# nicklashansen/tdmpc2

Hardware: AMD Instinct MI355X
Metric: plan() calls/sec (H=3, 512 samples, 6 iters) (higher is better)
Workload: dtype f32 (f16x2-split products: 22-bit operands, fp32 accumulate)

## Files before the change

tdmpc2_amd/csrc/common.cuh:

```cuda
#pragma once
#include <hip/hip_runtime.h>

#include <cmath>
#include <cstdint>
#include <cstdio>
#include <cstdlib>
#include <cstring>

#include "../../include/tdmpc2_plan.h"
#include "layer_route.h"
#include "plan_layout.h"
#include "fused_route.h"

typedef float f32x16 __attribute__((ext_vector_type(16)));
typedef float f32x4 __attribute__((ext_vector_type(4)));
typedef _Float16 f16x8 __attribute__((ext_vector_type(8)));
typedef _Float16 f16x4 __attribute__((ext_vector_type(4)));

namespace tdk {

constexpr int NTHREADS = 512;
constexpr float LN_EPS = 1e-5f;

constexpr int GBN = 128;
// ... 40 lines not shown
__device__ __forceinline__ void raise_fault(unsigned int *err, unsigned int code) {
    __hip_atomic_store(err, code, __ATOMIC_RELAXED, __HIP_MEMORY_SCOPE_SYSTEM);
    __hip_atomic_store(err + 8, 1u, __ATOMIC_RELAXED, __HIP_MEMORY_SCOPE_SYSTEM);
}

struct RefitParams {
    int E, N, H, A, K, iter, last, eval_mode;
    int Nvalid;
    int stage;
    float temperature, min_std, max_std;
    float *value;
    const float *actions;
    const float *act_mask;
    float *mean, *std;
    float *score;
    int *elite_idx;
    const float *gumbel_exp;
    const float *final_eps;
    unsigned long long seed;
    unsigned int call;
    float *prev_mean;
    float *action;
    const unsigned int *err;
    const unsigned int *err2;
    int regen, P, Apad;
    const float *sample_eps;
    long sample_eps_estride;
    float *dbg_value; long dbg_value_es;
    int *dbg_idx; long dbg_idx_es;
    float *dbg_score; long dbg_score_es;
    float *dbg_mean; long dbg_mean_es;
    float *dbg_std; long dbg_std_es;
};

struct RolloutParams {
    int E, N, H, A, Apad, P, stride, tiles, nq, num_bins, multitask, given_actions, iter, iters_total;
    int tile_off;
    int nnets;
    float log_std_min, log_std_dif;
    NetS dyn, rew, pi, term;
    NetS q[MAXQ];
    const float *bins;
    const float *z0;
    const float *beff;
    const float *cvec;
    const float *act_mask;
    const float *disc_pow;
    const float *mean;
    const float *std;
    const float *sample_eps;
    long sample_eps_estride;
    const float *pi_eps;
    long pi_eps_estride;
    const int *qidx;
    long qidx_estride;
    unsigned long long seed;
    unsigned int call;
    float *actions;
    float *value;
    float *zscratch;
    float *trace_tiles;
    float *trace_scalars;
    unsigned long long *timing;
    int fold_refit;
    unsigned int *ticket;
    RefitParams rf;
// ... 447 lines not shown
```

tdmpc2_amd/csrc/fused_kernels.cuh:

```cuda
#pragma once

#include "kloop_schedule.h"

#ifdef SPLIT_TIMING
#define TIMER_FIELDS mutable unsigned long long t_acc[14] = {0, 0, 0, 0, 0, 0, 0, 0, 0, 0, 0, 0, 0, 0}; mutable unsigned long long t_last = 0, t_begin = 0;
#define TIMER_START(c) { (c).t_last = (c).t_begin = __builtin_amdgcn_s_memtime(); }
#define TIMER_MARK(c, cls) { __builtin_amdgcn_sched_barrier(0); const unsigned long long t_now = __builtin_amdgcn_s_memtime(); __builtin_amdgcn_sched_barrier(0); (c).t_acc[cls] += t_now - (c).t_last; (c).t_last = t_now; }
#ifndef SPLIT_TIMING_WAVE
#define SPLIT_TIMING_WAVE 4
#endif
#define TIMER_FLUSH(c, ptr) if ((ptr) && threadIdx.x == 64 * SPLIT_TIMING_WAVE) { for (int i_ = 0; i_ < 14; ++i_) atomicAdd((ptr) + i_, (c).t_acc[i_]); atomicAdd((ptr) + 14, (c).t_last - (c).t_begin); atomicAdd((ptr) + 15, 1ull); }
#else
#define TIMER_FIELDS
#define TIMER_START(c)
#define TIMER_MARK(c, cls)
#define TIMER_FLUSH(c, ptr)
#endif
enum { T_KLOOP = 0, T_EPI = 1, T_HEAD = 2, T_ACT = 3, T_PARK = 4, T_TILE = 5, T_EPI_PRE = 6, T_EPI_SYNC = 7, T_EPI_BIAS = 8,
       T_EPI_COMB = 9, T_EPI_MATH = 10, T_CL_WAIT = 11, T_HEAD_K = 12, T_HEAD_ST = 13 };



#ifdef KS_NO_BIAS_LDS
constexpr bool KS_BIAS_LDS = false;
#else
constexpr bool KS_BIAS_LDS = true;
#endif
#ifdef KS_NO_ZH_REGS
constexpr bool KS_ZH_REGS = false;
#else
constexpr bool KS_ZH_REGS = true;
#endif
template <int APAD, int ST = 2, int NW = 8, int AR = 0>
struct CtxT {
    static constexpr bool BIAS_LDS = false;
    static constexpr int NST = ST;
    static constexpr int NWAVES = NW;
    static constexpr int ARITH = AR;
    static constexpr int FT = 16 / NW;
    static constexpr int NTHR = 64 * NW;
    static constexpr int TROWS = 32 * ST;
    static constexpr int SH = WIDTH + APAD;
    static constexpr int RSH = 2 * SH + 8;
    static constexpr int RSF_ = AR == 0 ? RSH / 2 : WIDTH + APAD + 4;
    static constexpr int KBLK = AR == 0 ? 16 : 8;
    static constexpr int ZKB = WIDTH / KBLK;
    _Float16 *act;
    float *stats;
    float *gb;
    int tid, wave, lane;
    mutable float pg[(WIDTH + NTHR - 1) / NTHR], pb[(WIDTH + NTHR - 1) / NTHR];
    TIMER_FIELDS
    __device__ __forceinline__ float *f32() const { return reinterpret_cast<float *>(act); }
    static constexpr __device__ __forceinline__ int RSF() { return RSF_; }
};
template <int APAD, int ST, int NW, int AR>
struct CtxPhT : CtxT<APAD, ST, NW, AR> {
    static constexpr bool BIAS_LDS = KS_BIAS_LDS;
    mutable float pbias = 0.f;
};

__device__ __forceinline__ float mish_fast(float x) {
    const float e = __expf(fminf(x, 20.f));
    const float n = e * (e + 2.f);
    return x * (n * __builtin_amdgcn_rcpf(n + 2.f));
}

template <class CT>
__device__ __forceinline__ float exp_a(float x) {
    if constexpr (CT::ARITH == 1) return expf(x);
    else return __expf(x);
}
template <class CT>
__device__ __forceinline__ float mish_a(float x) {
    if constexpr (CT::ARITH == 1) {
        const float e = expf(fminf(x, 20.f));
        const float n = e * (e + 2.f);
        return x * (n / (n + 2.f));
    } else {
        return mish_fast(x);
    }
}

__device__ __forceinline__ void split4(const f32x4 y, f16x4 &hi, f16x4 &lo, const float scale = ACT_SCALE) {
#pragma unroll
    for (int e = 0; e < 4; ++e) {
        const float ys = y[e] * scale;
        const _Float16 h = (_Float16)ys;
        hi[e] = h;
        lo[e] = (_Float16)(ys - (float)h);
    }
}


constexpr int PF = 2;
template <int FT>
struct BFragT {
    f16x8 h[FT], l[FT];
};
__device__ __forceinline__ f16x8 ldw(const char *ubase, unsigned voff, int imm) {
    return *reinterpret_cast<const f16x8 *>(ubase + voff + imm);
}
#define SPLIT_MFMA(a, b, c) __builtin_amdgcn_mfma_f32_32x32x16_f16(a, b, c, 0, 0, 0)
template <int FT>
__device__ __forceinline__ void load_b(BFragT<FT> &b, const char *u0, size_t ct_stride, unsigned voff) {
#pragma unroll
    for (int cc = 0; cc < FT; ++cc) {
        b.h[cc] = ldw(u0 + cc * ct_stride, voff, 0);
        b.l[cc] = ldw(u0 + cc * ct_stride, voff, 1024);
    }
}
template <int ST, int FT>
__device__ __forceinline__ void zero_acc(f32x16 (&a)[ST][FT]) {
#pragma unroll
    for (int r = 0; r < ST; ++r)
#pragma unroll
        for (int cc = 0; cc < FT; ++cc)
#pragma unroll
            for (int e = 0; e < 16; ++e) a[r][cc][e] = 0.f;
}
template <int ST>
struct AFragT {
    f16x8 h[ST], l[ST];
};
template <class CT>
__device__ __forceinline__ void load_a(AFragT<CT::NST> &a, const _Float16 *a0p, int kk) {
#pragma unroll
    for (int st = 0; st < CT::NST; ++st) {
        a.h[st] = *reinterpret_cast<const f16x8 *>(a0p + st * 32 * CT::RSH + kk * 16);
        a.l[st] = *reinterpret_cast<const f16x8 *>(a0p + st * 32 * CT::RSH + CT::SH + kk * 16);
    }
}
// ... 62 lines not shown
    a_dsrd<0>(a.h[0], la0);
    a_dsrd<2 * CT::SH>(a.l[0], la0);
    if constexpr (CT::NST == 2) {
        a_dsrd<0>(a.h[1], la1);
        a_dsrd<2 * CT::SH>(a.l[1], la1);
    }
}
__device__ __forceinline__ void a_load_w(BFragT<2> &b, unsigned voff, const char *s0, const char *s1) {
    asm volatile("s_nop 4\n\t"
                 "global_load_dwordx4 %0, %4, %5\n\t"
                 "global_load_dwordx4 %1, %4, %5 offset:1024\n\t"
                 "global_load_dwordx4 %2, %4, %6\n\t"
                 "global_load_dwordx4 %3, %4, %6 offset:1024"
                 : "=&v"(b.h[0]), "=&v"(b.l[0]), "=&v"(b.h[1]), "=&v"(b.l[1])
                 : "v"(voff), "s"(s0), "s"(s1));
}
template <class CT>
__device__ __forceinline__ void a_mfma12(f32x16 (&acc)[CT::NST][2], const BFragT<2> &w, const AFragT<CT::NST> &a) {
#pragma unroll
    for (int cc = 0; cc < 2; ++cc)
#pragma unroll
        for (int st = 0; st < CT::NST; ++st) A_MFMA(acc[st][cc], w.h[cc], a.h[st]);
#pragma unroll
    for (int cc = 0; cc < 2; ++cc)
#pragma unroll
        for (int st = 0; st < CT::NST; ++st) A_MFMA(acc[st][cc], w.l[cc], a.h[st]);
#pragma unroll
    for (int cc = 0; cc < 2; ++cc)
#pragma unroll
        for (int st = 0; st < CT::NST; ++st) A_MFMA(acc[st][cc], w.h[cc], a.l[st]);
}

template <class CT>
__device__ __forceinline__ void kloop_asm(const CT &c, const LayerS &ly, int kb0, int kb1, f32x16 (&acc)[CT::NST][2]) {
    static_assert(CT::FT == 2 && CT::ARITH == 0, "hand-ordered loop: 8-wave split-arithmetic geometry");
    const int i = c.lane & 31, hh = c.lane >> 5;
    unsigned la0 = lds_addr_of(c.act) + (unsigned)((i * CT::RSH + 8 * hh + kb0 * 16) * 2);
    unsigned la1 = la0 + 32 * CT::RSH * 2;
    const char *u0 = reinterpret_cast<const char *>(ly.wp) + ((size_t)(2 * c.wave) * ly.KB + kb0) * 2048;
    const size_t cts = (size_t)ly.KB * 2048;
    const unsigned voff = (unsigned)c.lane * 16u;
    const int nk = kb1 - kb0;
    constexpr int RD = KL_RD;
    BFragT<2> ring[RD];
    AFragT<CT::NST> a2[2];
#pragma unroll
    for (int d = 0; d < RD; ++d)
        if (d < nk) a_load_w(ring[d], voff, u0 + d * 2048, u0 + cts + d * 2048);
    a_load_act<CT>(a2[0], la0, la1);
    int k = 0;
    const char *pn = u0 + RD * 2048;
#pragma unroll 1
    for (; kl_steady_trip(k, nk, RD); k += RD) {
#pragma unroll
        for (int d = 0; d < RD; ++d) {
            asm volatile("s_waitcnt lgkmcnt(0)" ::: "memory");
            la0 += 32;
            la1 += 32;
            a_load_act<CT>(a2[(d & 1) ^ 1], la0, la1);
            asm volatile("s_waitcnt vmcnt(4)" ::: "memory");
            a_mfma12<CT>(acc, ring[d], a2[d & 1]);
            a_load_w(ring[d], voff, pn, pn + cts);
            pn += 2048;
        }
    }
#pragma unroll 1
    for (; k < nk; k += RD) {
#pragma unroll
        for (int d = 0; d < RD; ++d) {
            const int kk = k + d;
            if (kk < nk) {
                asm volatile("s_waitcnt lgkmcnt(0)" ::: "memory");
                if (kl_next_act(kk, nk)) {
                    la0 += 32;
                    la1 += 32;
                    a_load_act<CT>(a2[(d & 1) ^ 1], la0, la1);
                }
                const int behind = kl_behind(kk, nk, RD);
                if (behind >= 5) asm volatile("s_waitcnt vmcnt(20)" ::: "memory");
                else if (behind == 4) asm volatile("s_waitcnt vmcnt(16)" ::: "memory");
                else if (behind == 3) asm volatile("s_waitcnt vmcnt(12)" ::: "memory");
                else if (behind == 2) asm volatile("s_waitcnt vmcnt(8)" ::: "memory");
                else if (behind == 1) asm volatile("s_waitcnt vmcnt(4)" ::: "memory");
                else asm volatile("s_waitcnt vmcnt(0)" ::: "memory");
                a_mfma12<CT>(acc, ring[d], a2[d & 1]);
                if (kl_issue(kk, nk, RD)) {
                    a_load_w(ring[d], voff, pn, pn + cts);
                    pn += 2048;
                }
            }
        }
    }
    asm volatile("s_nop 7\n\ts_nop 7" ::: "memory");
}

template <class CT>
__device__ __forceinline__ void kloop_s(const CT &c, const LayerS &ly, int kb0, int kb1, f32x16 (&acc)[CT::NST][CT::FT]) {
    if constexpr (CT::ARITH == 1) {
        kloop_f32(c, ly, kb0, kb1, acc);
        return;
    }
    if constexpr (CT::ARITH == 0 && CT::FT == 2) {
        kloop_asm(c, ly, kb0, kb1, acc);
        return;
    }
    constexpr int FT = CT::FT;
    constexpr int PFD = FT == 2 ? PF : (PF > 1 ? PF / 2 : 1);
    const int i = c.lane & 31, hh = c.lane >> 5;
    const _Float16 *a0p = c.act + i * c.RSH + 8 * hh + kb0 * 16;
    const char *u0 = reinterpret_cast<const char *>(ly.wp) + ((size_t)(FT * c.wave) * ly.KB + kb0) * 2048;
    const size_t cts = (size_t)ly.KB * 2048;
    unsigned voff = (unsigned)c.lane * 16u;
    asm volatile("" : "+v"(voff));
    const int nk = kb1 - kb0;
    BFragT<FT> ring[PFD];
#pragma unroll
    for (int d = 0; d < PFD; ++d) {
        const int kd = d < nk ? d : nk - 1;
        load_b(ring[d], u0 + (size_t)kd * 2048, cts, voff);
    }
    AFragT<CT::NST> an;
    load_a<CT>(an, a0p, 0);
    __builtin_amdgcn_sched_barrier(0);
#pragma unroll 1
    for (int k = 0; k < nk; k += PFD) {
#pragma unroll
        for (int d = 0; d < PFD; ++d) {
            const int kk = k + d;
            if (kk < nk) {
                const AFragT<CT::NST> a = an;
                load_a<CT>(an, a0p, kk + 1 < nk ? kk + 1 : kk);
#pragma unroll
                for (int cc = 0; cc < FT; ++cc)
#pragma unroll
                    for (int st = 0; st < CT::NST; ++st) acc[st][cc] = SPLIT_MFMA(ring[d].h[cc], a.h[st], acc[st][cc]);
#pragma unroll
// ... 163 lines not shown
        _Float16 *hp = c.act + (32 * st + j) * c.RSH + 32 * CT::FT * c.wave + 4 * hh;
#pragma unroll
        for (int ft = 0; ft < CT::FT; ++ft)
#pragma unroll
            for (int m = 0; m < 4; ++m) {
                f32x4 v;
#pragma unroll
                for (int r = 0; r < 4; ++r) v[r] = y[st][ft][4 * m + r];
                f16x4 hi, lo;
                split4(v, hi, lo, scale);
                *reinterpret_cast<f16x4 *>(hp + 32 * ft + 8 * m) = hi;
                *reinterpret_cast<f16x4 *>(hp + c.SH + 32 * ft + 8 * m) = lo;
            }
    }
}

struct GB {
    const float *g = nullptr, *b = nullptr, *bias = nullptr;
};
__device__ __forceinline__ GB gb_of(const LayerS &ly) { return GB{ly.g, ly.b, ly.bias}; }
__device__ __forceinline__ GB gb_of(const LayerS &ly, const float *bias) { return GB{ly.g, ly.b, bias}; }

template <class CT>
__device__ __forceinline__ void gb_prefetch(const CT &c, const float *g, const float *b) {
#pragma unroll
    for (int u = 0; u < (WIDTH + CT::NTHR - 1) / CT::NTHR; ++u) {
        const int f = c.tid + u * CT::NTHR;
        c.pg[u] = f < WIDTH ? g[f] : 0.f;
        c.pb[u] = f < WIDTH ? b[f] : 0.f;
    }
}
template <class CT>
__device__ __forceinline__ void gb_prefetch(const CT &c, const GB next) {
    gb_prefetch(c, next.g, next.b);
    if constexpr (CT::BIAS_LDS) {
        static_assert(CT::FT == 2 && CT::NTHR == WIDTH, "thread tid fetches feature tid of its own wave's 64");
        c.pbias = next.bias[c.tid];
    }
}
template <class CT>
__device__ __forceinline__ void gb_commit(const CT &c) {
    if constexpr (CT::BIAS_LDS) c.stats[c.wave * (CT::TROWS * 2) + c.lane] = c.pbias;
#pragma unroll
    for (int u = 0; u < (WIDTH + CT::NTHR - 1) / CT::NTHR; ++u) {
        const int f = c.tid + u * CT::NTHR;
        if (f < WIDTH) {
            c.gb[f] = c.pg[u];
            c.gb[WIDTH + f] = c.pb[u];
        }
    }
}
template <class CT>
__device__ __forceinline__ void epi_barrier(const CT &c) {
    __syncthreads();
    gb_commit(c);
}

enum { EPI_PRE = 1, EPI_MATH = 2, EPI_STORE = 4, EPI_ALL = 7 };
template <int ACT, class CT, bool HASBIAS = true, int PIECES = EPI_ALL>
__device__ __forceinline__ void epi_t(const CT &c, f32x16 (&acc)[CT::NST][CT::FT], float osc, float asc, const float *bias,
                                      GB next, float *zcopy) {
    constexpr int FT = CT::FT, NW = CT::NWAVES;
    constexpr float CNT = 32.f * FT;
    const int j = c.lane & 31, hh = c.lane >> 5;
    const int poff = 32 * FT * c.wave + 4 * hh;
    if constexpr (PIECES & EPI_PRE) {
// ... 161 lines not shown

template <class CT>
__device__ __forceinline__ float twohot_rows_s(const CT &c, const float *bins, int num_bins) {
    const int part = c.tid & 7;
    const bool live = (c.tid >> 3) < CT::TROWS;
    const int row = live ? c.tid >> 3 : 0;
    const float *rp = c.f32() + row * c.RSF();
    if (num_bins <= 1) {
        const float x1 = rp[0];
        return num_bins == 0 ? x1 : symexp_f(x1);
    }
    float v[16];
    float m = -INFINITY;
#pragma unroll
    for (int q = 0; q < 16; ++q) {
        const int jj = part + 8 * q;
        v[q] = (jj < num_bins) ? rp[jj] : -INFINITY;
        m = fmaxf(m, v[q]);
    }
    m = group_max<8>(m);
    float es = 0.f, x = 0.f;
#pragma unroll
    for (int q = 0; q < 16; ++q) {
        const int jj = part + 8 * q;
        const float ev = (jj < num_bins) ? expf(v[q] - m) : 0.f;
        es += ev;
        x = fmaf(ev, (jj < num_bins) ? bins[jj] : 0.f, x);
    }
    es = group_sum<8>(es);
    x = group_sum<8>(x);
    return symexp_f(x / es);
}

template <int ACT, class CT>
__device__ __forceinline__ void layer_full_s(const CT &c, const LayerS &ly, const float *bias, int kb0, int kb1,
                                             GB next, float *zcopy = nullptr) {
    f32x16 acc[CT::NST][CT::FT];
    zero_acc(acc);
    if (next.g) gb_prefetch(c, next);
    kloop_s(c, ly, kb0, kb1, acc);
    TIMER_MARK(c, T_KLOOP)
    epi_t<ACT>(c, acc, *ly.oscale, *ly.ascale, bias, next, zcopy);
    epi_barrier(c);
    TIMER_MARK(c, T_EPI)
}
template <int ACT, class CT>
__device__ __forceinline__ void layer_held_s(const CT &c, const LayerS &ly, const float *bias, int kb0, int kb1, GB next,
                                             f32x16 (&acc)[CT::NST][CT::FT]) {
    zero_acc(acc);
    if (next.g) gb_prefetch(c, next);
    kloop_s(c, ly, kb0, kb1, acc);
    TIMER_MARK(c, T_KLOOP)
    epi_t<ACT>(c, acc, *ly.oscale, *ly.ascale, bias, next, nullptr);
    epi_barrier(c);
    TIMER_MARK(c, T_EPI)
}

template <class CT>
__device__ __forceinline__ void head_logits_s(const CT &c, const LayerS &ly) {
    f32x16 acc[CT::NST];
    const float osc = *ly.oscale;
    const int ct = c.wave;
    if (ct < ly.CT) kloop_tile_s(c, ly, ct, 0, CT::ZKB, acc);
    __syncthreads();
    TIMER_MARK(c, T_HEAD_K)
    if (ct < ly.CT) {
#pragma unroll
        for (int rt = 0; rt < CT::NST; ++rt) store_tile_s(c, acc[rt], osc, ly.bias, ct, rt);
    }
    __syncthreads();
    TIMER_MARK(c, T_HEAD_ST)
}

template <class CT>
__device__ __forceinline__ float head_twohot_s(const CT &c, const LayerS &ly, const float *bins, int num_bins) {
    head_logits_s(c, ly);
    const float r = twohot_rows_s(c, bins, num_bins);
    __syncthreads();
    return r;
}

template <class CT>
__device__ __forceinline__ void put_action(const CT &c, int row, int a, float v) {
    if constexpr (CT::ARITH == 1) {
        c.f32()[row * CT::RSF() + WIDTH + a] = v;
        return;
    }
    const float vs = v * ACT_SCALE;
    const _Float16 h = (_Float16)vs;
    _Float16 *rp = c.act + row * c.RSH + WIDTH + a;
    rp[0] = h;
    rp[c.SH] = (_Float16)(vs - (float)h);
}

template <class CT, typename EpsFn>
__device__ __forceinline__ void head_pi_rows_s(const CT &c, int A, int Apad, float lsmin, float lsdif, const float *mask_wg, EpsFn eps,
                                               float *gdst, int nvalid, float *tsc, const float *mask_tab = nullptr,
                                               const int *row_task = nullptr, int put_rows = CT::TROWS, bool agent_store = false);

template <class CT, typename EpsFn>
__device__ __forceinline__ void head_pi_s(const CT &c, const LayerS &ly, int A, int Apad, float lsmin, float lsdif,
                                          const float *mask_wg, EpsFn eps, float *gdst, int nvalid, float *tsc,
                                          const float *mask_tab = nullptr, const int *row_task = nullptr) {
    head_logits_s(c, ly);
    head_pi_rows_s(c, A, Apad, lsmin, lsdif, mask_wg, eps, gdst, nvalid, tsc, mask_tab, row_task, CT::TROWS, false);
}

template <class CT, typename EpsFn>
__device__ __forceinline__ void head_pi_rows_s(const CT &c, int A, int Apad, float lsmin, float lsdif, const float *mask_wg, EpsFn eps,
                                               float *gdst, int nvalid, float *tsc, const float *mask_tab, const int *row_task,
// ... 234 lines not shown
#pragma unroll
        for (int u = 0; u < 2; ++u) {
            const int a = a0 + u;
            if (a < p.A) {
                if (!sampled) {
                    v[u] = ag[(size_t)n * p.A + a];
                } else {
                    float r = z[u];
                    if (p.sample_eps)
                        r = p.sample_eps[(size_t)e * p.sample_eps_estride +
                                         (unsigned)(((size_t)t * (p.N - p.P) + (n - p.P)) * p.A + a)];
                    v[u] = sample_action(sm_mean[t * p.A + a], sm_std[t * p.A + a], r);
                }
                if (mask && !p.given_actions) v[u] *= mask[a];
                if (!p.given_actions) ag[(size_t)n * p.A + a] = v[u];
            }
            put_action(c, row, a, v[u]);
        }
    }
}

#define DUMP_TILE(...) do { if constexpr (TRACE) dump_tile_s(__VA_ARGS__); } while (0)
template <int APAD, int ST, int NW, int AR, int EP, int TR = 0>
__global__ __launch_bounds__(64 * NW, 2) void ks_rollout(RolloutParams p) {
    constexpr bool TRACE = TR || EP;
    extern __shared__ __attribute__((aligned(16))) float smem[];
    __shared__ int s_is_last;
    const int e = blockIdx.x / p.tiles, tile = p.tile_off + blockIdx.x % p.tiles;
    const int tid = threadIdx.x;
    typedef CtxPhT<APAD, ST, NW, AR> CT;
    constexpr int TROWS = CT::TROWS, NTHR = CT::NTHR, FT = CT::FT;
    constexpr int ZKB16 = CT::ZKB;
    constexpr bool ZH_REGS = !EP && KS_ZH_REGS;
    CT c{{reinterpret_cast<_Float16 *>(smem), smem + TROWS * CT::RSF(), smem + TROWS * CT::RSF() + 1024, tid,
          __builtin_amdgcn_readfirstlane(tid >> 6), tid & 63}};
    float *sm_mean = smem + TROWS * CT::RSF() + 2048;
    float *sm_std = sm_mean + p.H * p.A;
    const int row0 = tile * TROWS;
    const float *mask = p.act_mask ? p.act_mask + (size_t)e * p.A : nullptr;
    const float *disc = p.disc_pow + (size_t)e * (p.H + 1);
    const int KBA = ZKB16 + p.Apad / CT::KBLK;
    float *zs = p.zscratch + (size_t)blockIdx.x * TROWS * WIDTH;
    const int NSLOT = 5 * p.H + 7;
    const bool live = (tid >> 3) < TROWS;
    float *tsc = nullptr;
    if constexpr (TRACE) tsc = p.trace_scalars && live ? p.trace_scalars + ((size_t)e * p.N + row0 + (tid >> 3)) * (p.H + 2 + p.A) : nullptr;

    for (int idx = tid; idx < p.H * p.A; idx += NTHR) {
        sm_mean[idx] = p.mean[(size_t)e * p.H * p.A + idx];
        sm_std[idx] = p.std[(size_t)e * p.H * p.A + idx];
    }
    int q0, q1;
    if (p.qidx) {
        q0 = p.qidx[(size_t)e * p.qidx_estride + 0];
        q1 = p.qidx[(size_t)e * p.qidx_estride + 1];
    } else {
        const uint4 r = rng_raw(p.seed, p.call, SITE_QIDX, p.iter, e, 0);
        q0 = (int)(r.x % (unsigned)p.nq);
        q1 = (int)(r.y % (unsigned)(p.nq - 1));
        if (q1 >= q0) ++q1;
    }
    const float *b_rew = p.multitask ? p.beff + ((size_t)e * p.nnets + BE_REW) * WIDTH : p.rew.l[0].bias;
    const float *b_dyn = p.multitask ? p.beff + ((size_t)e * p.nnets + BE_DYN) * WIDTH : p.dyn.l[0].bias;
    const float *b_pi = p.multitask ? p.beff + ((size_t)e * p.nnets + BE_PI) * WIDTH : p.pi.l[0].bias;
    const float *b_q0 = p.multitask ? p.beff + ((size_t)e * p.nnets + BE_Q0 + q0) * WIDTH : p.q[q0].l[0].bias;
    const float *b_q1 = p.multitask ? p.beff + ((size_t)e * p.nnets + BE_Q0 + q1) * WIDTH : p.q[q1].l[0].bias;
    const float *c_rew = p.cvec + ((size_t)e * 2 + 0) * WIDTH, *c_dyn = p.cvec + ((size_t)e * 2 + 1) * WIDTH;
    gb_prefetch(c, gb_of(p.rew.l[0], c_rew));
    epi_barrier(c);

    float G = 0.f;
    float termv = 0.f;
    TIMER_START(c)
    for (int t = 0; t < p.H; ++t) {
        sample_actions(c, p, e, row0, mask, sm_mean, sm_std, t);
        __syncthreads();
        TIMER_MARK(c, T_ACT)
        const bool term_step = EP && t > 0;
        f32x16 accd[ST][FT];
        {
            f32x16 acc[ST][FT];
            gb_prefetch(c, gb_of(p.rew.l[1]));
            first_layers_s(c, p.dyn.l[0], p.rew.l[0], t == 0 ? ZKB16 : 0, KBA, accd, acc);
            TIMER_MARK(c, T_KLOOP)
            if constexpr (EP) {
                if (term_step) {
                    park(c, accd, zs);
                    zero_acc(accd);
                    kloop_s(c, p.term.l[0], 0, ZKB16, accd);
                }
            }
            epi_t<0>(c, acc, *p.rew.l[0].oscale, *p.rew.l[0].ascale, t == 0 ? c_rew : b_rew, gb_of(p.rew.l[1]), nullptr);
        }
        epi_barrier(c);
        TIMER_MARK(c, T_EPI)
        DUMP_TILE(c, p.trace_tiles, NSLOT, 5 * t + 0, p.rew.l[0].ascale);
        layer_full_s<0>(c, p.rew.l[1], p.rew.l[1].bias, 0, ZKB16,
                        term_step ? gb_of(p.term.l[0]) : gb_of(p.dyn.l[0], t == 0 ? c_dyn : b_dyn));
        DUMP_TILE(c, p.trace_tiles, NSLOT, 5 * t + 1, p.rew.l[1].ascale);
        if (term_step) gb_prefetch(c, gb_of(p.term.l[1]));
        else gb_prefetch(c, gb_of(p.dyn.l[1]));
        const float r = head_twohot_s(c, p.rew.l[2], p.bins, p.num_bins);
        TIMER_MARK(c, T_HEAD)
        if (tsc && (tid & 7) == 0) tsc[t] = r;
        if constexpr (EP) {
            if (term_step) {
                epi_t<0>(c, accd, *p.term.l[0].oscale, *p.term.l[0].ascale, p.term.l[0].bias, gb_of(p.term.l[1]), nullptr);
                epi_barrier(c);
                layer_full_s<0>(c, p.term.l[1], p.term.l[1].bias, 0, ZKB16, gb_of(p.dyn.l[0], b_dyn));
                gb_prefetch(c, gb_of(p.dyn.l[1]));
                termv = fminf(termv + head_term_s(c, p.term.l[2]), 1.f);
                unpark(c, accd, zs);
            }
        }
        G += disc[t] * (1.f - termv) * r;
        epi_t<0>(c, accd, *p.dyn.l[0].oscale, *p.dyn.l[0].ascale, t == 0 ? c_dyn : b_dyn, gb_of(p.dyn.l[1]), nullptr);
        epi_barrier(c);
        TIMER_MARK(c, T_EPI)
        DUMP_TILE(c, p.trace_tiles, NSLOT, 5 * t + 2, p.dyn.l[0].ascale);
        layer_full_s<0>(c, p.dyn.l[1], p.dyn.l[1].bias, 0, ZKB16, gb_of(p.dyn.l[2]));
        DUMP_TILE(c, p.trace_tiles, NSLOT, 5 * t + 3, p.dyn.l[1].ascale);
        if constexpr (ZH_REGS) {
            if (t == p.H - 1) break;
            layer_full_s<1>(c, p.dyn.l[2], p.dyn.l[2].bias, 0, ZKB16, gb_of(p.rew.l[0], b_rew), nullptr);
        } else {
            layer_full_s<1>(c, p.dyn.l[2], p.dyn.l[2].bias, 0, ZKB16,
                            t == p.H - 1 ? gb_of(p.pi.l[0], b_pi) : gb_of(p.rew.l[0], b_rew), t == p.H - 1 ? zs : nullptr);
        }
        DUMP_TILE(c, p.trace_tiles, NSLOT, 5 * t + 4);
    }
    f32x16 acch[ST][FT];
    if constexpr (ZH_REGS) {
        layer_held_s<1>(c, p.dyn.l[2], p.dyn.l[2].bias, 0, ZKB16, gb_of(p.pi.l[0], b_pi), acch);
        DUMP_TILE(c, p.trace_tiles, NSLOT, 5 * (p.H - 1) + 4);
    }
    if constexpr (EP) {
        zero_acc(acch);
        kloop_s(c, p.term.l[0], 0, ZKB16, acch);
    }
    layer_full_s<0>(c, p.pi.l[0], b_pi, 0, ZKB16, gb_of(p.pi.l[1]));
    DUMP_TILE(c, p.trace_tiles, NSLOT, 5 * p.H + 0, p.pi.l[0].ascale);
    layer_full_s<0>(c, p.pi.l[1], p.pi.l[1].bias, 0, ZKB16, EP ? gb_of(p.term.l[0]) : gb_of(p.q[q0].l[0], b_q0));
    DUMP_TILE(c, p.trace_tiles, NSLOT, 5 * p.H + 1, p.pi.l[1].ascale);
    if constexpr (EP) gb_prefetch(c, gb_of(p.term.l[1]));
    {
        auto eps = [&](int row, int a) -> float {
            const unsigned ridx = (unsigned)((size_t)(row0 + row) * p.A + a);
            if (p.pi_eps) return p.pi_eps[(size_t)e * p.pi_eps_estride + ridx];
            return rng_normal(p.seed, p.call, SITE_PI, p.iter, e, ridx);
        };
        head_pi_s(c, p.pi.l[2], p.A, p.Apad, p.log_std_min, p.log_std_dif, mask, eps, nullptr, 0,
                  tsc ? tsc + p.H + 2 : nullptr);
    }
    TIMER_MARK(c, T_HEAD)
    if constexpr (EP) {
        epi_t<0>(c, acch, *p.term.l[0].oscale, *p.term.l[0].ascale, p.term.l[0].bias, gb_of(p.term.l[1]), nullptr);
        epi_barrier(c);
        layer_full_s<0>(c, p.term.l[1], p.term.l[1].bias, 0, ZKB16, gb_of(p.q[q0].l[0], b_q0));
        termv = fminf(termv + head_term_s(c, p.term.l[2]), 1.f);
    }
    if constexpr (ZH_REGS) regs_to_tile(c, acch);
    else tile_from_global_s(c, zs);
    __syncthreads();
    TIMER_MARK(c, T_TILE)
    DUMP_TILE(c, p.trace_tiles, NSLOT, 5 * p.H + 2);
    {
        f32x16 acc[ST][FT];
        gb_prefetch(c, gb_of(p.q[q0].l[1]));
        first_layers_s(c, p.q[q1].l[0], p.q[q0].l[0], 0, KBA, acch, acc);
        TIMER_MARK(c, T_KLOOP)
        epi_t<0>(c, acc, *p.q[q0].l[0].oscale, *p.q[q0].l[0].ascale, b_q0, gb_of(p.q[q0].l[1]), nullptr);
    }
    epi_barrier(c);
    TIMER_MARK(c, T_EPI)
    DUMP_TILE(c, p.trace_tiles, NSLOT, 5 * p.H + 3, p.q[q0].l[0].ascale);
    layer_full_s<0>(c, p.q[q0].l[1], p.q[q0].l[1].bias, 0, ZKB16, gb_of(p.q[q1].l[0], b_q1));
    DUMP_TILE(c, p.trace_tiles, NSLOT, 5 * p.H + 4, p.q[q0].l[1].ascale);
    gb_prefetch(c, gb_of(p.q[q1].l[1]));
    const float qa = head_twohot_s(c, p.q[q0].l[2], p.bins, p.num_bins);
    TIMER_MARK(c, T_HEAD)
    epi_t<0>(c, acch, *p.q[q1].l[0].oscale, *p.q[q1].l[0].ascale, b_q1, gb_of(p.q[q1].l[1]), nullptr);
    epi_barrier(c);
    TIMER_MARK(c, T_EPI)
    DUMP_TILE(c, p.trace_tiles, NSLOT, 5 * p.H + 5, p.q[q1].l[0].ascale);
    layer_full_s<0>(c, p.q[q1].l[1], p.q[q1].l[1].bias, 0, ZKB16, GB{});
    DUMP_TILE(c, p.trace_tiles, NSLOT, 5 * p.H + 6, p.q[q1].l[1].ascale);
    const float qb = head_twohot_s(c, p.q[q1].l[2], p.bins, p.num_bins);
    TIMER_MARK(c, T_HEAD)
    TIMER_FLUSH(c, p.timing)
    if (tsc && (tid & 7) == 0) {
        tsc[p.H] = qa;
        tsc[p.H + 1] = qb;
    }
    const float val = G + disc[p.H] * (1.f - termv) * ((qa + qb) / 2.f);
    if (!p.fold_refit) {
        if ((tid & 7) == 0 && live) p.value[(size_t)e * p.N + row0 + (tid >> 3)] = val;
        return;
    }
    if ((tid & 7) == 0 && live)
        __hip_atomic_store(p.value + (size_t)e * p.N + row0 + (tid >> 3), val, __ATOMIC_RELAXED, __HIP_MEMORY_SCOPE_AGENT);
    asm volatile("s_waitcnt vmcnt(0)" ::: "memory");
    __builtin_amdgcn_fence(__ATOMIC_RELEASE, "workgroup");
    __syncthreads();
    if (tid == 0) {
        const unsigned old = __hip_atomic_fetch_add(p.ticket + e, 1u, __ATOMIC_RELAXED, __HIP_MEMORY_SCOPE_AGENT);
        const int last = old == (unsigned)(p.tiles - 1);
        if (last) __hip_atomic_store(p.ticket + e, 0u, __ATOMIC_RELAXED, __HIP_MEMORY_SCOPE_AGENT);
        s_is_last = last;
    }
    __syncthreads();
    if (!s_is_last) return;
    refit_plan(p.rf, e, smem, tid, NTHR);
}

template <int APAD, int AR>
__global__ __launch_bounds__(NTHREADS, 2) void ks_value(ValueParams p) {
    extern __shared__ __attribute__((aligned(16))) float smem[];
    const int tid = threadIdx.x;
// ... 73 lines not shown
```

tdmpc2_amd/csrc/kloop_schedule.h:

```cpp
#pragma once

#ifndef __HIPCC__
#ifndef __host__
#define __host__
#endif
#ifndef __device__
#define __device__
#endif
#endif

constexpr int KL_RD = 2;
constexpr int KL_W_LOADS = 4;

__host__ __device__ inline bool kl_steady_trip(int k, int nk, int rd) { return k + 2 * rd - 1 < nk; }
__host__ __device__ inline int kl_steady_vmcnt(int rd) { return KL_W_LOADS * (rd - 1); }
__host__ __device__ inline int kl_behind(int kk, int nk, int rd) { return nk - 1 - kk < rd - 1 ? nk - 1 - kk : rd - 1; }
__host__ __device__ inline bool kl_next_act(int kk, int nk) { return kk + 1 < nk; }
__host__ __device__ inline bool kl_issue(int kk, int nk, int rd) { return kk + rd < nk; }
```

tdmpc2_amd/csrc/tdmpc2_plan.hip:

```cpp
#include <cstdarg>
#include <cstring>
#include <new>

#include "handle.h"
#include "launch.h"

namespace {

__global__ void k_refit(RefitParams p) {
    extern __shared__ __attribute__((aligned(16))) float smem[];
    refit_plan(p, blockIdx.x, smem, threadIdx.x, blockDim.x);
}

}
int tdk::launch_refit(const RefitParams &fp, int E, int N, size_t lds, hipStream_t st) {
    hipLaunchKernelGGL(k_refit, dim3(E), dim3(refit_threads(N)), lds, st, fp);
    LAUNCH_CHECK();
    return 0;
}
namespace {

__global__ void ks_task_bias(TaskBiasParams p) {
    const int task = blockIdx.x, f = threadIdx.x;
    const float *emb = p.task_emb + (size_t)task * p.T;
// ... 651 lines not shown
        L.side = sr.stream; L.ev_fork = sr.ev[0]; L.ev_side = sr.ev[1]; L.ev_xread = sr.ev[2];
    }
    if (lo.err_line && (rc = err_line_create(h))) return rc;
    if (hipEventCreateWithFlags(&h->turn_ev, hipEventDisableTiming) != hipSuccess) {
        h->turn_ev = nullptr;
        return fail(TDMPC2_ERR_HIP, "hipEventCreate failed");
    }
    if (pl_set_lds()) return TDMPC2_ERR_HIP;
    if (!L.on) {
        const int ar = h->split ? 0 : 1;
        rc = fused_ops(h->Apad).set_lds(ar, c.episodic, h->lds_bytes);
        if (!rc) rc = model_ops(h->Apad).set_lds(ar, h->lds_bytes);
        if (!rc) rc = policy_loss_ops(h->Apad).set_lds(ar, h->lds_bytes);
        if (!rc && h->cl_max_clusters) rc = cluster_ops(h->Apad).set_lds(c.episodic, h->cl_lds);
        if (rc) return TDMPC2_ERR_HIP;
    }
    if (L.on && h->split) {
        L.fuse_ln = env.fuse_ln;
        L.ksplit = env.ksplit;
        L.mid = env.fewrow;
        if ((rc = ksws_ensure(h, L.ksplit))) return rc;
        if (env.gw_timing) {
            if ((rc = dev_alloc(h, (void **)&L.gw_timing, 32 * 8))) return rc;
            if (hipMemset(L.gw_timing, 0, 32 * 8) != hipSuccess) return fail(TDMPC2_ERR_HIP, "hipMemset failed");
        }
    }
    h->cluster_mode = env.cluster;
    h->user_cluster_mode = h->cluster_mode;
    h->user_fuse_ln = L.fuse_ln;
#ifdef TDMPC2_TEST_HOOKS
    if (const char *cf = getenv("TDMPC2_CLUSTER_FAULT")) h->cl_fault = atoi(cf);
#endif
    if (h->cl_fault) L.mid = false;
    if (env.timing && dev_alloc(h, (void **)&h->timing, 16 * 8) == 0) (void)hipMemset(h->timing, 0, 16 * 8);
    undo.h = nullptr;
    *out = h;
    return TDMPC2_OK;
}

void tdmpc2_plan_destroy(tdmpc2_plan_t *h) {
    if (!h) return;
    DevGuard dev_(h->cfg.device);
    if (h->timing) {
        unsigned long long t[16];
        if (hipMemcpy(t, h->timing, sizeof t, hipMemcpyDeviceToHost) == hipSuccess && t[15] > 0) {
            static const char *names[16] = {"kloop", "epi_post", "head", "actions", "park/unpark", "tile_from_global", "epi_stats", "epi_sync",
                                            "epi_bias", "epi_combine", "epi_math_store", "cluster_wait", "head_kloop", "head_stage", "total", "workgroups"};
            fprintf(stderr, "[tdmpc2_plan timing max_envs=%d] mean cycles per workgroup (one wave, SPLIT_TIMING_WAVE):", h->cfg.max_envs);
            for (int i = 0; i < 15; ++i)
                if (names[i][0]) fprintf(stderr, " %s=%.0f", names[i], (double)t[i] / (double)t[15]);
            fprintf(stderr, "\n");
        }
    }
    if (h->lay.gw_timing) {
        unsigned long long t[32];
        if (hipDeviceSynchronize() == hipSuccess && hipMemcpy(t, h->lay.gw_timing, sizeof t, hipMemcpyDeviceToHost) == hipSuccess) {
            static const char *cls[4] = {"mish K<1024", "mish K>=1024", "simnorm K<1024", "simnorm K>=1024"};
            for (int c = 0; c < 4; ++c) {
                const unsigned long long *q = t + 8 * c;
                if (!q[6]) continue;
                const double n = (double)q[6];
                fprintf(stderr, "[g_gemm_w timing max_envs=%d, %s] workgroups=%llu mean cycles of wave 0: loop_end=%.0f stats_stored=%.0f "
                        "peers_arrived=%.0f row_stats=%.0f end=%.0f\n", h->cfg.max_envs, cls[c], q[6], q[1] / n, q[2] / n, q[3] / n, q[4] / n, q[5] / n);
            }
        }
    }
    if (h->lay.side) {
        SideRes sr;
        sr.stream = h->lay.side; sr.ev[0] = h->lay.ev_fork; sr.ev[1] = h->lay.ev_side; sr.ev[2] = h->lay.ev_xread;
        side_release(h->cfg.device, sr);
    }
    for (void *p : h->allocs) (void)hipFree(p);
    if (h->cl_err_host) (void)hipHostFree(h->cl_err_host);
    for (hipEvent_t e : h->ev) (void)hipEventDestroy(e);
    if (h->turn_ev) (void)hipEventDestroy(h->turn_ev);
    delete h;
}

uint64_t tdmpc2_plan_device_bytes(const tdmpc2_plan_t *h) { return h ? h->bytes : 0; }
int tdmpc2_plan_path(const tdmpc2_plan_t *h) { return h ? h->cfg.path : -1; }
int tdmpc2_plan_precision(const tdmpc2_plan_t *h) { return h ? h->cfg.precision : -1; }

namespace {
// ... 1504 lines not shown
```

Before: 10350.

## Prefetch next layer's weight ring during epilogue across layer seams

Moves the initial weight-block ring loads of the hand-ordered k-loop into a per-context ring that is issued during the previous layer's epilogue, before the barrier, so global weight loads for the next layer overlap epilogue math and the sync. It also loads gamma/beta/bias prefetch with a single per-thread address (SEAM_ADDR) instead of the generic path. It extends split timing with new counter classes. The ring now lives across function boundaries, which raises register pressure and risks spills or lower occupancy.

```diff
diff --git a/tdmpc2_amd/csrc/common.cuh b/tdmpc2_amd/csrc/common.cuh
--- a/tdmpc2_amd/csrc/common.cuh
+++ b/tdmpc2_amd/csrc/common.cuh
@@ -96,6 +96,8 @@
     float *dbg_mean; long dbg_mean_es;
     float *dbg_std; long dbg_std_es;
 };
+
+constexpr int T_NCLS = 17;
 
 struct RolloutParams {
     int E, N, H, A, Apad, P, stride, tiles, nq, num_bins, multitask, given_actions, iter, iters_total;
diff --git a/tdmpc2_amd/csrc/fused_kernels.cuh b/tdmpc2_amd/csrc/fused_kernels.cuh
--- a/tdmpc2_amd/csrc/fused_kernels.cuh
+++ b/tdmpc2_amd/csrc/fused_kernels.cuh
@@ -3,13 +3,13 @@
 #include "kloop_schedule.h"
 
 #ifdef SPLIT_TIMING
-#define TIMER_FIELDS mutable unsigned long long t_acc[14] = {0, 0, 0, 0, 0, 0, 0, 0, 0, 0, 0, 0, 0, 0}; mutable unsigned long long t_last = 0, t_begin = 0;
+#define TIMER_FIELDS mutable unsigned long long t_acc[T_NCLS] = {}; mutable unsigned long long t_last = 0, t_begin = 0;
 #define TIMER_START(c) { (c).t_last = (c).t_begin = __builtin_amdgcn_s_memtime(); }
 #define TIMER_MARK(c, cls) { __builtin_amdgcn_sched_barrier(0); const unsigned long long t_now = __builtin_amdgcn_s_memtime(); __builtin_amdgcn_sched_barrier(0); (c).t_acc[cls] += t_now - (c).t_last; (c).t_last = t_now; }
 #ifndef SPLIT_TIMING_WAVE
 #define SPLIT_TIMING_WAVE 4
 #endif
-#define TIMER_FLUSH(c, ptr) if ((ptr) && threadIdx.x == 64 * SPLIT_TIMING_WAVE) { for (int i_ = 0; i_ < 14; ++i_) atomicAdd((ptr) + i_, (c).t_acc[i_]); atomicAdd((ptr) + 14, (c).t_last - (c).t_begin); atomicAdd((ptr) + 15, 1ull); }
+#define TIMER_FLUSH(c, ptr) if ((ptr) && threadIdx.x == 64 * SPLIT_TIMING_WAVE) { for (int i_ = 0; i_ < T_NCLS; ++i_) atomicAdd((ptr) + i_, (c).t_acc[i_]); atomicAdd((ptr) + T_NCLS, (c).t_last - (c).t_begin); atomicAdd((ptr) + T_NCLS + 1, 1ull); }
 #else
 #define TIMER_FIELDS
 #define TIMER_START(c)
@@ -17,7 +17,9 @@
 #define TIMER_FLUSH(c, ptr)
 #endif
 enum { T_KLOOP = 0, T_EPI = 1, T_HEAD = 2, T_ACT = 3, T_PARK = 4, T_TILE = 5, T_EPI_PRE = 6, T_EPI_SYNC = 7, T_EPI_BIAS = 8,
-       T_EPI_COMB = 9, T_EPI_MATH = 10, T_CL_WAIT = 11, T_HEAD_K = 12, T_HEAD_ST = 13 };
+       T_EPI_COMB = 9, T_EPI_MATH = 10, T_CL_WAIT = 11, T_HEAD_K = 12, T_HEAD_ST = 13,
+       T_KLOOP_HEAD = 14, T_EPI_OSC = 15, T_TWOHOT = 16 };
+static_assert(T_TWOHOT + 1 == T_NCLS, "common.cuh: T_NCLS counters + total + workgroups");
 
 
 
@@ -31,9 +33,24 @@
 #else
 constexpr bool KS_ZH_REGS = true;
 #endif
+#ifdef KS_NO_SEAM_WARM
+constexpr bool KS_SEAM_RING = false;
+#else
+constexpr bool KS_SEAM_RING = true;
+#endif
+#ifdef KS_NO_SEAM_ADDR
+constexpr bool KS_SEAM_ADDR = false;
+#else
+constexpr bool KS_SEAM_ADDR = true;
+#endif
+template <int FT>
+struct BFragT {
+    f16x8 h[FT], l[FT];
+};
 template <int APAD, int ST = 2, int NW = 8, int AR = 0>
 struct CtxT {
     static constexpr bool BIAS_LDS = false;
+    static constexpr bool SEAM_RING = false, SEAM_ADDR = false;
     static constexpr int NST = ST;
     static constexpr int NWAVES = NW;
     static constexpr int ARITH = AR;
@@ -57,7 +74,10 @@
 template <int APAD, int ST, int NW, int AR>
 struct CtxPhT : CtxT<APAD, ST, NW, AR> {
     static constexpr bool BIAS_LDS = KS_BIAS_LDS;
+    static constexpr bool SEAM_RING = KS_SEAM_RING && AR == 0 && NW == 8;
+    static constexpr bool SEAM_ADDR = KS_SEAM_ADDR;
     mutable float pbias = 0.f;
+    mutable BFragT<2> ring[KL_RD];
 };
 
 __device__ __forceinline__ float mish_fast(float x) {
@@ -94,10 +114,6 @@
 
 
 constexpr int PF = 2;
-template <int FT>
-struct BFragT {
-    f16x8 h[FT], l[FT];
-};
 __device__ __forceinline__ f16x8 ldw(const char *ubase, unsigned voff, int imm) {
     return *reinterpret_cast<const f16x8 *>(ubase + voff + imm);
 }
@@ -226,8 +242,26 @@
 }
 
 template <class CT>
+__device__ __forceinline__ void ring_issue(const CT &c, const LayerS &ly, int kb0, int kb1) {
+    static_assert(CT::SEAM_RING && CT::FT == 2 && CT::ARITH == 0, "the hand-ordered loop's ring");
+    const char *wp = reinterpret_cast<const char *>(ly.wp);
+    const unsigned voff = (unsigned)c.lane * 16u;
+    const int nk = kb1 - kb0;
+#pragma unroll
+    for (int d = 0; d < KL_RD; ++d)
+        if (kl_ring_fill(d, nk, KL_RD))
+            a_load_w(c.ring[d], voff, wp + kl_block_offset(2 * c.wave, ly.KB, kb0 + d), wp + kl_block_offset(2 * c.wave + 1, ly.KB, kb0 + d));
+}
+template <bool PRE, class CT>
+__device__ __forceinline__ auto &ring_of(const CT &c, BFragT<2> (&local)[KL_RD]) {
+    if constexpr (PRE) return c.ring;
+    else return local;
+}
+
+template <class CT, bool PRE = false>
 __device__ __forceinline__ void kloop_asm(const CT &c, const LayerS &ly, int kb0, int kb1, f32x16 (&acc)[CT::NST][2]) {
     static_assert(CT::FT == 2 && CT::ARITH == 0, "hand-ordered loop: 8-wave split-arithmetic geometry");
+    TIMER_MARK(c, T_KLOOP)
     const int i = c.lane & 31, hh = c.lane >> 5;
     unsigned la0 = lds_addr_of(c.act) + (unsigned)((i * CT::RSH + 8 * hh + kb0 * 16) * 2);
     unsigned la1 = la0 + 32 * CT::RSH * 2;
@@ -236,12 +270,20 @@
     const unsigned voff = (unsigned)c.lane * 16u;
     const int nk = kb1 - kb0;
     constexpr int RD = KL_RD;
-    BFragT<2> ring[RD];
+    BFragT<2> lring[RD];
+    BFragT<2> (&ring)[RD] = ring_of<PRE>(c, lring);
     AFragT<CT::NST> a2[2];
-#pragma unroll
-    for (int d = 0; d < RD; ++d)
-        if (d < nk) a_load_w(ring[d], voff, u0 + d * 2048, u0 + cts + d * 2048);
+    if constexpr (!PRE) {
+#pragma unroll
+        for (int d = 0; d < RD; ++d)
+            if (kl_ring_fill(d, nk, RD)) a_load_w(ring[d], voff, u0 + d * 2048, u0 + cts + d * 2048);
+    }
     a_load_act<CT>(a2[0], la0, la1);
+#ifdef SPLIT_TIMING
+    if (nk > 1) asm volatile("s_waitcnt lgkmcnt(0)\n\ts_waitcnt vmcnt(4)" ::: "memory");
+    else asm volatile("s_waitcnt lgkmcnt(0)\n\ts_waitcnt vmcnt(0)" ::: "memory");
+    TIMER_MARK(c, T_KLOOP_HEAD)
+#endif
     int k = 0;
     const char *pn = u0 + RD * 2048;
 #pragma unroll 1
@@ -288,14 +330,15 @@
     asm volatile("s_nop 7\n\ts_nop 7" ::: "memory");
 }
 
-template <class CT>
+template <class CT, bool PRE = false>
 __device__ __forceinline__ void kloop_s(const CT &c, const LayerS &ly, int kb0, int kb1, f32x16 (&acc)[CT::NST][CT::FT]) {
+    static_assert(!PRE || (CT::ARITH == 0 && CT::FT == 2), "only the hand-ordered loop takes a ring requested ahead");
     if constexpr (CT::ARITH == 1) {
         kloop_f32(c, ly, kb0, kb1, acc);
         return;
     }
     if constexpr (CT::ARITH == 0 && CT::FT == 2) {
-        kloop_asm(c, ly, kb0, kb1, acc);
+        kloop_asm<CT, PRE>(c, ly, kb0, kb1, acc);
         return;
     }
     constexpr int FT = CT::FT;
@@ -525,6 +568,15 @@
 }
 template <class CT>
 __device__ __forceinline__ void gb_prefetch(const CT &c, const GB next) {
+    if constexpr (CT::BIAS_LDS && CT::SEAM_ADDR) {
+        static_assert(CT::FT == 2 && CT::NTHR == WIDTH, "thread tid fetches feature tid of its own wave's 64");
+        unsigned f = (unsigned)c.tid;
+        asm volatile("" : "+v"(f));
+        c.pg[0] = next.g[f];
+        c.pb[0] = next.b[f];
+        c.pbias = next.bias[f];
+        return;
+    }
     gb_prefetch(c, next.g, next.b);
     if constexpr (CT::BIAS_LDS) {
         static_assert(CT::FT == 2 && CT::NTHR == WIDTH, "thread tid fetches feature tid of its own wave's 64");
@@ -752,26 +804,38 @@
     return symexp_f(x / es);
 }
 
-template <int ACT, class CT>
+#ifdef SPLIT_TIMING
+#define TIMER_MARK_SCALARS(c) { asm volatile("s_waitcnt lgkmcnt(0)" ::: "memory"); TIMER_MARK(c, T_EPI_OSC) }
+#else
+#define TIMER_MARK_SCALARS(c)
+#endif
+
+template <int ACT, class CT, bool PRE = false, bool NK = false>
 __device__ __forceinline__ void layer_full_s(const CT &c, const LayerS &ly, const float *bias, int kb0, int kb1,
-                                             GB next, float *zcopy = nullptr) {
+                                             GB next, float *zcopy = nullptr, const LayerS *nxk = nullptr) {
     f32x16 acc[CT::NST][CT::FT];
     zero_acc(acc);
     if (next.g) gb_prefetch(c, next);
-    kloop_s(c, ly, kb0, kb1, acc);
+    kloop_s<CT, PRE>(c, ly, kb0, kb1, acc);
     TIMER_MARK(c, T_KLOOP)
-    epi_t<ACT>(c, acc, *ly.oscale, *ly.ascale, bias, next, zcopy);
+    const float osc = *ly.oscale, asc = *ly.ascale;
+    TIMER_MARK_SCALARS(c)
+    epi_t<ACT>(c, acc, osc, asc, bias, next, zcopy);
+    if constexpr (NK) ring_issue(c, *nxk, 0, CT::ZKB);
     epi_barrier(c);
     TIMER_MARK(c, T_EPI)
 }
-template <int ACT, class CT>
+template <int ACT, class CT, bool PRE = false, bool NK = false>
 __device__ __forceinline__ void layer_held_s(const CT &c, const LayerS &ly, const float *bias, int kb0, int kb1, GB next,
-                                             f32x16 (&acc)[CT::NST][CT::FT]) {
+                                             f32x16 (&acc)[CT::NST][CT::FT], const LayerS *nxk = nullptr) {
     zero_acc(acc);
     if (next.g) gb_prefetch(c, next);
-    kloop_s(c, ly, kb0, kb1, acc);
+    kloop_s<CT, PRE>(c, ly, kb0, kb1, acc);
     TIMER_MARK(c, T_KLOOP)
-    epi_t<ACT>(c, acc, *ly.oscale, *ly.ascale, bias, next, nullptr);
+    const float osc = *ly.oscale, asc = *ly.ascale;
+    TIMER_MARK_SCALARS(c)
+    epi_t<ACT>(c, acc, osc, asc, bias, next, nullptr);
+    if constexpr (NK) ring_issue(c, *nxk, 0, CT::ZKB);
     epi_barrier(c);
     TIMER_MARK(c, T_EPI)
 }
@@ -796,6 +860,7 @@
 __device__ __forceinline__ float head_twohot_s(const CT &c, const LayerS &ly, const float *bins, int num_bins) {
     head_logits_s(c, ly);
     const float r = twohot_rows_s(c, bins, num_bins);
+    TIMER_MARK(c, T_TWOHOT)
     __syncthreads();
     return r;
 }
@@ -1096,6 +1161,7 @@
     constexpr int TROWS = CT::TROWS, NTHR = CT::NTHR, FT = CT::FT;
     constexpr int ZKB16 = CT::ZKB;
     constexpr bool ZH_REGS = !EP && KS_ZH_REGS;
+    constexpr bool SR = CT::SEAM_RING;
     CT c{{reinterpret_cast<_Float16 *>(smem), smem + TROWS * CT::RSF(), smem + TROWS * CT::RSF() + 1024, tid,
           __builtin_amdgcn_readfirstlane(tid >> 6), tid & 63}};
     float *sm_mean = smem + TROWS * CT::RSF() + 2048;
@@ -1156,11 +1222,12 @@
             }
             epi_t<0>(c, acc, *p.rew.l[0].oscale, *p.rew.l[0].ascale, t == 0 ? c_rew : b_rew, gb_of(p.rew.l[1]), nullptr);
         }
+        if constexpr (SR) ring_issue(c, p.rew.l[1], 0, ZKB16);
         epi_barrier(c);
         TIMER_MARK(c, T_EPI)
         DUMP_TILE(c, p.trace_tiles, NSLOT, 5 * t + 0, p.rew.l[0].ascale);
-        layer_full_s<0>(c, p.rew.l[1], p.rew.l[1].bias, 0, ZKB16,
-                        term_step ? gb_of(p.term.l[0]) : gb_of(p.dyn.l[0], t == 0 ? c_dyn : b_dyn));
+        layer_full_s<0, CT, SR>(c, p.rew.l[1], p.rew.l[1].bias, 0, ZKB16,
+                                term_step ? gb_of(p.term.l[0]) : gb_of(p.dyn.l[0], t == 0 ? c_dyn : b_dyn));
         DUMP_TILE(c, p.trace_tiles, NSLOT, 5 * t + 1, p.rew.l[1].ascale);
         if (term_step) gb_prefetch(c, gb_of(p.term.l[1]));
         else gb_prefetch(c, gb_of(p.dyn.l[1]));
@@ -1179,32 +1246,33 @@
         }
         G += disc[t] * (1.f - termv) * r;
         epi_t<0>(c, accd, *p.dyn.l[0].oscale, *p.dyn.l[0].ascale, t == 0 ? c_dyn : b_dyn, gb_of(p.dyn.l[1]), nullptr);
+        if constexpr (SR) ring_issue(c, p.dyn.l[1], 0, ZKB16);
         epi_barrier(c);
         TIMER_MARK(c, T_EPI)
         DUMP_TILE(c, p.trace_tiles, NSLOT, 5 * t + 2, p.dyn.l[0].ascale);
-        layer_full_s<0>(c, p.dyn.l[1], p.dyn.l[1].bias, 0, ZKB16, gb_of(p.dyn.l[2]));
+        layer_full_s<0, CT, SR, SR>(c, p.dyn.l[1], p.dyn.l[1].bias, 0, ZKB16, gb_of(p.dyn.l[2]), nullptr, &p.dyn.l[2]);
         DUMP_TILE(c, p.trace_tiles, NSLOT, 5 * t + 3, p.dyn.l[1].ascale);
         if constexpr (ZH_REGS) {
             if (t == p.H - 1) break;
-            layer_full_s<1>(c, p.dyn.l[2], p.dyn.l[2].bias, 0, ZKB16, gb_of(p.rew.l[0], b_rew), nullptr);
+            layer_full_s<1, CT, SR>(c, p.dyn.l[2], p.dyn.l[2].bias, 0, ZKB16, gb_of(p.rew.l[0], b_rew), nullptr);
         } else {
-            layer_full_s<1>(c, p.dyn.l[2], p.dyn.l[2].bias, 0, ZKB16,
-                            t == p.H - 1 ? gb_of(p.pi.l[0], b_pi) : gb_of(p.rew.l[0], b_rew), t == p.H - 1 ? zs : nullptr);
+            layer_full_s<1, CT, SR>(c, p.dyn.l[2], p.dyn.l[2].bias, 0, ZKB16,
+                                    t == p.H - 1 ? gb_of(p.pi.l[0], b_pi) : gb_of(p.rew.l[0], b_rew), t == p.H - 1 ? zs : nullptr);
         }
         DUMP_TILE(c, p.trace_tiles, NSLOT, 5 * t + 4);
     }
     f32x16 acch[ST][FT];
     if constexpr (ZH_REGS) {
-        layer_held_s<1>(c, p.dyn.l[2], p.dyn.l[2].bias, 0, ZKB16, gb_of(p.pi.l[0], b_pi), acch);
+        layer_held_s<1, CT, SR, SR>(c, p.dyn.l[2], p.dyn.l[2].bias, 0, ZKB16, gb_of(p.pi.l[0], b_pi), acch, &p.pi.l[0]);
         DUMP_TILE(c, p.trace_tiles, NSLOT, 5 * (p.H - 1) + 4);
     }
     if constexpr (EP) {
         zero_acc(acch);
         kloop_s(c, p.term.l[0], 0, ZKB16, acch);
     }
-    layer_full_s<0>(c, p.pi.l[0], b_pi, 0, ZKB16, gb_of(p.pi.l[1]));
+    layer_full_s<0, CT, SR && ZH_REGS, SR>(c, p.pi.l[0], b_pi, 0, ZKB16, gb_of(p.pi.l[1]), nullptr, &p.pi.l[1]);
     DUMP_TILE(c, p.trace_tiles, NSLOT, 5 * p.H + 0, p.pi.l[0].ascale);
-    layer_full_s<0>(c, p.pi.l[1], p.pi.l[1].bias, 0, ZKB16, EP ? gb_of(p.term.l[0]) : gb_of(p.q[q0].l[0], b_q0));
+    layer_full_s<0, CT, SR>(c, p.pi.l[1], p.pi.l[1].bias, 0, ZKB16, EP ? gb_of(p.term.l[0]) : gb_of(p.q[q0].l[0], b_q0));
     DUMP_TILE(c, p.trace_tiles, NSLOT, 5 * p.H + 1, p.pi.l[1].ascale);
     if constexpr (EP) gb_prefetch(c, gb_of(p.term.l[1]));
     {
@@ -1235,19 +1303,21 @@
         TIMER_MARK(c, T_KLOOP)
         epi_t<0>(c, acc, *p.q[q0].l[0].oscale, *p.q[q0].l[0].ascale, b_q0, gb_of(p.q[q0].l[1]), nullptr);
     }
+    if constexpr (SR) ring_issue(c, p.q[q0].l[1], 0, ZKB16);
     epi_barrier(c);
     TIMER_MARK(c, T_EPI)
     DUMP_TILE(c, p.trace_tiles, NSLOT, 5 * p.H + 3, p.q[q0].l[0].ascale);
-    layer_full_s<0>(c, p.q[q0].l[1], p.q[q0].l[1].bias, 0, ZKB16, gb_of(p.q[q1].l[0], b_q1));
+    layer_full_s<0, CT, SR>(c, p.q[q0].l[1], p.q[q0].l[1].bias, 0, ZKB16, gb_of(p.q[q1].l[0], b_q1));
     DUMP_TILE(c, p.trace_tiles, NSLOT, 5 * p.H + 4, p.q[q0].l[1].ascale);
     gb_prefetch(c, gb_of(p.q[q1].l[1]));
     const float qa = head_twohot_s(c, p.q[q0].l[2], p.bins, p.num_bins);
     TIMER_MARK(c, T_HEAD)
     epi_t<0>(c, acch, *p.q[q1].l[0].oscale, *p.q[q1].l[0].ascale, b_q1, gb_of(p.q[q1].l[1]), nullptr);
+    if constexpr (SR) ring_issue(c, p.q[q1].l[1], 0, ZKB16);
     epi_barrier(c);
     TIMER_MARK(c, T_EPI)
     DUMP_TILE(c, p.trace_tiles, NSLOT, 5 * p.H + 5, p.q[q1].l[0].ascale);
-    layer_full_s<0>(c, p.q[q1].l[1], p.q[q1].l[1].bias, 0, ZKB16, GB{});
+    layer_full_s<0, CT, SR>(c, p.q[q1].l[1], p.q[q1].l[1].bias, 0, ZKB16, GB{});
     DUMP_TILE(c, p.trace_tiles, NSLOT, 5 * p.H + 6, p.q[q1].l[1].ascale);
     const float qb = head_twohot_s(c, p.q[q1].l[2], p.bins, p.num_bins);
     TIMER_MARK(c, T_HEAD)
diff --git a/tdmpc2_amd/csrc/kloop_schedule.h b/tdmpc2_amd/csrc/kloop_schedule.h
--- a/tdmpc2_amd/csrc/kloop_schedule.h
+++ b/tdmpc2_amd/csrc/kloop_schedule.h
@@ -12,6 +12,9 @@
 constexpr int KL_RD = 2;
 constexpr int KL_W_LOADS = 4;
 
+__host__ __device__ inline bool kl_ring_fill(int d, int nk, int rd) { return d < rd && d < nk; }
+constexpr long KL_BLOCK_BYTES = 2048;
+__host__ __device__ inline long kl_block_offset(int tile, int KB, int kb) { return ((long)tile * KB + kb) * KL_BLOCK_BYTES; }
 __host__ __device__ inline bool kl_steady_trip(int k, int nk, int rd) { return k + 2 * rd - 1 < nk; }
 __host__ __device__ inline int kl_steady_vmcnt(int rd) { return KL_W_LOADS * (rd - 1); }
 __host__ __device__ inline int kl_behind(int kk, int nk, int rd) { return nk - 1 - kk < rd - 1 ? nk - 1 - kk : rd - 1; }
diff --git a/tdmpc2_amd/csrc/tdmpc2_plan.hip b/tdmpc2_amd/csrc/tdmpc2_plan.hip
--- a/tdmpc2_amd/csrc/tdmpc2_plan.hip
+++ b/tdmpc2_amd/csrc/tdmpc2_plan.hip
@@ -707,7 +707,7 @@
     if (const char *cf = getenv("TDMPC2_CLUSTER_FAULT")) h->cl_fault = atoi(cf);
 #endif
     if (h->cl_fault) L.mid = false;
-    if (env.timing && dev_alloc(h, (void **)&h->timing, 16 * 8) == 0) (void)hipMemset(h->timing, 0, 16 * 8);
+    if (env.timing && dev_alloc(h, (void **)&h->timing, (T_NCLS + 2) * 8) == 0) (void)hipMemset(h->timing, 0, (T_NCLS + 2) * 8);
     undo.h = nullptr;
     *out = h;
     return TDMPC2_OK;
@@ -717,13 +717,14 @@
     if (!h) return;
     DevGuard dev_(h->cfg.device);
     if (h->timing) {
-        unsigned long long t[16];
-        if (hipMemcpy(t, h->timing, sizeof t, hipMemcpyDeviceToHost) == hipSuccess && t[15] > 0) {
-            static const char *names[16] = {"kloop", "epi_post", "head", "actions", "park/unpark", "tile_from_global", "epi_stats", "epi_sync",
-                                            "epi_bias", "epi_combine", "epi_math_store", "cluster_wait", "head_kloop", "head_stage", "total", "workgroups"};
+        unsigned long long t[T_NCLS + 2];
+        if (hipMemcpy(t, h->timing, sizeof t, hipMemcpyDeviceToHost) == hipSuccess && t[T_NCLS + 1] > 0) {
+            static const char *names[T_NCLS + 2] = {"kloop", "epi_post", "head", "actions", "park/unpark", "tile_from_global", "epi_stats", "epi_sync",
+                                                    "epi_bias", "epi_combine", "epi_math_store", "cluster_wait", "head_kloop", "head_stage",
+                                                    "kloop_head", "epi_oscale", "twohot_rows", "total", "workgroups"};
             fprintf(stderr, "[tdmpc2_plan timing max_envs=%d] mean cycles per workgroup (one wave, SPLIT_TIMING_WAVE):", h->cfg.max_envs);
-            for (int i = 0; i < 15; ++i)
-                if (names[i][0]) fprintf(stderr, " %s=%.0f", names[i], (double)t[i] / (double)t[15]);
+            for (int i = 0; i < T_NCLS + 1; ++i)
+                if (names[i][0]) fprintf(stderr, " %s=%.0f", names[i], (double)t[i] / (double)t[T_NCLS + 1]);
             fprintf(stderr, "\n");
         }
     }
```

Measured after the change: 10390 (median of 6 runs). No clear change (+0.4%).
